# brade31919/radar_depth

Hardware: AMD Instinct MI355X
Metric: training samples/sec, resnet18_latefusion b=16 450x800 rgbd, 1/2/4/8 MI355X (higher is better)
Workload: dtype f32

## Files before the change

radar_depth_amd/csrc/gconv_split.hip:

```cpp
#include <math.h>
#include <stdlib.h>

#include <mutex>
#include <string>
#include <type_traits>
#include <unordered_map>
#include <vector>

#include "common.h"
#include "slot_map.h"

namespace rd {

typedef __bf16 sbf16x8 __attribute__((ext_vector_type(8)));
typedef unsigned int su32x4 __attribute__((ext_vector_type(4)));

constexpr unsigned GS_OOB = 0x80000000u;
constexpr int GS_CKP = 16;
constexpr int GS_PSB = (GS_CKP + 8) * 2;
constexpr int GS_UPP = 6;
constexpr int GS_UW = 2;
constexpr int GS_TPS = 3;

struct GsArgs {
    RdConvDesc d;
    const float* in;
    const unsigned short* w;
    float* out;
    const float* addend;
    const float* bias;
    float* stat;
    int act, act_cols, ld_add, ldw;
    int TH, TW, PP, tiles_total, n_cotiles, taps_max;
    int vec4;
    int pplane;
    long long wplane;
    int tapoff[RD_MAX_PHASES][RD_MAX_TAPS];
    unsigned long long* trace;
    int trace_role;
    const unsigned short* inp;
    long long xplane;
    long long mpix;
    int kplane;
    int stagger;
    int dbg;
    int ppitch[RD_MAX_PHASES];
    const int* slots;
    const float* bnb_x;
    const float* bnb_scale;
    const float* bnb_shift;
    const float* bnb_mean;
    int bnb_ld, bnb_act;
};

__device__ __forceinline__ void vm_wait_upto(int n) {
#define RD_VMW(k) case k: asm volatile("s_waitcnt vmcnt(" #k ") lgkmcnt(0)" ::: "memory"); break;
    switch (n < 47 ? n : 47) {
        RD_VMW(0) RD_VMW(1) RD_VMW(2) RD_VMW(3) RD_VMW(4) RD_VMW(5) RD_VMW(6) RD_VMW(7) RD_VMW(8) RD_VMW(9) RD_VMW(10) RD_VMW(11)
        RD_VMW(12) RD_VMW(13) RD_VMW(14) RD_VMW(15) RD_VMW(16) RD_VMW(17) RD_VMW(18) RD_VMW(19) RD_VMW(20) RD_VMW(21) RD_VMW(22) RD_VMW(23)
        RD_VMW(24) RD_VMW(25) RD_VMW(26) RD_VMW(27) RD_VMW(28) RD_VMW(29) RD_VMW(30) RD_VMW(31) RD_VMW(32) RD_VMW(33) RD_VMW(34) RD_VMW(35)
        RD_VMW(36) RD_VMW(37) RD_VMW(38) RD_VMW(39) RD_VMW(40) RD_VMW(41) RD_VMW(42) RD_VMW(43) RD_VMW(44) RD_VMW(45) RD_VMW(46) RD_VMW(47)
    }
#undef RD_VMW
}

typedef float sf32x2 __attribute__((ext_vector_type(2)));
typedef __bf16 sbf16x2 __attribute__((ext_vector_type(2)));
__device__ __forceinline__ unsigned cvt_pk(float a, float b) {
    sf32x2 v;
    v[0] = a; v[1] = b;
    return __builtin_bit_cast(unsigned, __builtin_convertvector(v, sbf16x2));
}
__device__ __forceinline__ void split8(const float4 v0, const float4 v1, sbf16x8& p0, sbf16x8& p1, sbf16x8& p2) {
    const float x[8] = {v0.x, v0.y, v0.z, v0.w, v1.x, v1.y, v1.z, v1.w};
    su32x4 w0, w1, w2;
#pragma unroll
    for (int i = 0; i < 4; ++i) {
        float a = x[2 * i], b = x[2 * i + 1];
        const unsigned u0 = cvt_pk(a, b);
        a -= __uint_as_float(u0 << 16);
        b -= __uint_as_float(u0 & 0xffff0000u);
        const unsigned u1 = cvt_pk(a, b);
        a -= __uint_as_float(u1 << 16);
        b -= __uint_as_float(u1 & 0xffff0000u);
        w0[i] = u0;
        w1[i] = u1;
        w2[i] = cvt_pk(a, b);
    }
    p0 = __builtin_bit_cast(sbf16x8, w0);
    p1 = __builtin_bit_cast(sbf16x8, w1);
    p2 = __builtin_bit_cast(sbf16x8, w2);
}

template <int MT, int NT, bool PDB, bool PRE, bool BNB = false>
__global__ __launch_bounds__(512) void gconv_split_kernel(const GsArgs a) {
    static_assert(!PRE || PDB, "the pre-split form copies the next chunk's patch while the current one is read: two patch buffers");
    constexpr int BM = 4 * MT * 32;
    constexpr int BN = NT * 32;
    constexpr int LBN = NT == 2 ? 6 : 5;
    extern __shared__ __attribute__((aligned(16))) float smem[];
    const int tid = threadIdx.x, lane = tid & 63;
    const int wave = __builtin_amdgcn_readfirstlane(tid >> 6);
    const bool loader = wave >= 4;
    const int wm = wave & 3;
    const int l31 = lane & 31, hh = lane >> 5;
    const RdConvDesc& D = a.d;

    if (a.trace && tid == 0) a.trace[(size_t)blockIdx.x * 64 + 62] = __builtin_readcyclecounter();
    const int vid = xcd_remap(blockIdx.x, gridDim.x);
    const int cot = vid % a.n_cotiles;
    const int pt = vid / a.n_cotiles;
    const int n = pt / a.tiles_total;
    const int tt = pt - n * a.tiles_total;
    int ph_ = 0;
    for (int i = 1; i < D.n_phases; ++i)
        if (tt >= D.phase[i].tile_begin) ph_ = i;
    const int ph = __builtin_amdgcn_readfirstlane(ph_);
    const RdPhase& P = D.phase[ph];
    const int tloc = tt - P.tile_begin;
    const int tiles_w = (P.lw + a.TW - 1) / a.TW;
    const int r0 = (tloc / tiles_w) * a.TH, c0 = (tloc % tiles_w) * a.TW;
    const int th_n = min(a.TH, P.lh - r0), tw_n = min(a.TW, P.lw - c0);
    const int IS = D.in_stride, OS = D.out_stride;
    const int PW = (a.TW - 1) * IS + (P.dw_max - P.dw_min) + 1;
    const int PWP = a.ppitch[ph];
    const int PH = (th_n - 1) * IS + (P.dh_max - P.dh_min) + 1;
    const int ih0 = r0 * IS + P.dh_min, iw0 = c0 * IS + P.dw_min;
    const int ntaps = __builtin_amdgcn_readfirstlane(P.n_taps);
    const int ngroups = (ntaps + GS_TPS - 1) / GS_TPS;
    const int co0 = cot * BN;

    int* s_opix = reinterpret_cast<int*>(smem);
    int* s_apix = s_opix + BM;
    int* s_widx = s_apix + BM;
    char* s_w = reinterpret_cast<char*>(s_widx + 32);
    constexpr int WPP = GS_TPS * 2 * BN * 16;
    constexpr int SLAB = 3 * WPP;
    char* s_patch = s_w + 3 * SLAB;
    const int pplane = a.pplane;

    for (int m = tid; m < BM; m += 512) {
        const int sv = a.slots[ph * BM + m];
        const bool have = sv >= 0;
        const int r = sv >> 16, c = sv & 0xffff, rho = -1 - sv;
        const bool ok = have && (r < th_n) && (c < tw_n);
        s_opix[m] = ok ? ((n * D.Ho + (r0 + r) * OS + P.out_off_h) * D.Wo + (c0 + c) * OS + P.out_off_w) : -1;
        s_apix[m] = have ? ((r * IS) * PWP + c * IS) : rho * IS;
    }
    if (tid < ntaps) s_widx[tid] = P.widx[tid];
    if constexpr (PRE) {
        const int n16 = (2 * 3 * pplane) >> 4;
        for (int e = tid; e < n16; e += 512) *reinterpret_cast<uint4*>(s_patch + (size_t)e * 16) = make_uint4(0u, 0u, 0u, 0u);
    }
    rd_sync();

    f32x16 acc[MT][NT];

    const int nchunks = D.Cin / GS_CKP;
    const int total_groups = nchunks * ngroups;
    const char* in_n = reinterpret_cast<const char*>(a.in) + (size_t)n * D.Hi * D.Wi * D.ldi * 4;
    const unsigned img_bytes = (unsigned)(D.Hi * D.Wi * D.ldi) * 4u;
    const int rowu = PW * 2;
    const int nseg = (rowu + 63) >> 6;
    const int nsegs = PH * nseg;
    auto unit_of = [&](int seg, unsigned& goff, int& ldst) {
        const int row = nseg == 1 ? seg : seg / nseg;
        const int cu = ((seg - row * nseg) << 6) + lane;
        const int px = cu >> 1, qq = cu & 1;
        const int ih = ih0 + row, iw = iw0 + px;
        const bool ok = seg < nsegs && cu < rowu;
        ldst = ok ? (row * PWP + px) * GS_PSB + qq * 16 : -1;
        goff = (ok && ih >= 0 && ih < D.Hi && iw >= 0 && iw < D.Wi) ? (unsigned)(((ih * D.Wi + iw) * D.ldi + qq * 8) * 4) : GS_OOB;
    };
    auto stage_first_chunk = [&]() {
        constexpr int UP8 = (GS_UPP + 1) / 2;
        const __amdgpu_buffer_rsrc_t r = __builtin_amdgcn_make_buffer_rsrc(const_cast<char*>(in_n), 0, img_bytes, 0x00020000);
        float4 f0[UP8], f1[UP8];
        int dst[UP8];
#pragma unroll
        for (int u = 0; u < UP8; ++u) {
            unsigned go;
            unit_of(wave + 8 * u, go, dst[u]);
            f0[u] = __builtin_bit_cast(float4, __builtin_amdgcn_raw_buffer_load_b128(r, (int)go, 0, 0));
            f1[u] = __builtin_bit_cast(float4, __builtin_amdgcn_raw_buffer_load_b128(r, (int)go + 16, 0, 0));
        }
        const unsigned base = (unsigned)(size_t)s_patch;
#pragma unroll
        for (int u = 0; u < UP8; ++u) {
            sbf16x8 q0, q1, q2;
            split8(f0[u], f1[u], q0, q1, q2);
            if (dst[u] >= 0) {
                const su32x4 d0 = __builtin_bit_cast(su32x4, q0), d1 = __builtin_bit_cast(su32x4, q1), d2 = __builtin_bit_cast(su32x4, q2);
                const unsigned ad = base + dst[u];
                asm volatile("ds_write_b128 %0, %1" ::"v"(ad), "v"(d0) : "memory");
                asm volatile("ds_write_b128 %0, %1" ::"v"(ad + pplane), "v"(d1) : "memory");
                asm volatile("ds_write_b128 %0, %1" ::"v"(ad + 2 * pplane), "v"(d2) : "memory");
            }
            __builtin_amdgcn_sched_barrier(0);
        }
    };

    if (loader) {
        const int ltid = tid - 256;
        const int lw = wave - 4;
        const int cin8 = D.Cin >> 3;
        unsigned pgo[GS_UPP];
        int pdst[GS_UPP];
        if constexpr (!PRE) {
#pragma unroll
            for (int u = 0; u < GS_UPP; ++u) unit_of(lw + 4 * u, pgo[u], pdst[u]);
        }
        auto issue_patch = [&](int pbuf, int blk) -> int {
            int cnt = 0;
            if (a.dbg & 8) return 0;
            const char* src0 = reinterpret_cast<const char*>(a.inp) + ((size_t)blk * a.mpix + (size_t)n * D.Hi * D.Wi) * 32;
            char* dst0 = s_patch + pbuf * 3 * pplane;
            const int nsg = (PW + 63) >> 6;
            for (int r = lw; r < PH; r += 4) {
                const int ih = ih0 + r;
                if (ih < 0 || ih >= D.Hi) continue;
                for (int sg = 0; sg < nsg; ++sg) {
                    const int col = (sg << 6) + lane, iw = iw0 + col;
                    const bool ok = col < PW && iw >= 0 && iw < D.Wi;
                    if (!__any(ok)) continue;
                    const char* src = src0 + ((size_t)ih * D.Wi + iw) * 32;
                    char* dst = dst0 + ((size_t)r * PWP + (sg << 6)) * 16;
                    if (ok) {
#pragma unroll
                        for (int p = 0; p < 3; ++p)
#pragma unroll
                            for (int u = 0; u < 2; ++u)
                                glds16(reinterpret_cast<const float*>(src + p * a.xplane + u * 16), reinterpret_cast<float*>(dst + p * pplane + u * a.kplane));
                    }
                    cnt += 6;
                }
            }
            return cnt;
        };
        auto issue_slab = [&](int buf, int cb, int g) -> int {
            if (a.dbg & 4) return 0;
            int cnt = 0;
            const int tap0 = g * GS_TPS;
            constexpr int welems = (GS_TPS * 2) << LBN;
            const char* src = reinterpret_cast<const char*>(a.w) + (size_t)(cb >> 3) * a.ldw * 16;
            char* dst = s_w + buf * SLAB;
#pragma unroll
            for (int u = 0; u < GS_UW; ++u) {
                const int e = ltid + u * 256;
                if (e < welems) {
                    const int j = e & (BN - 1), tk = e >> LBN;
                    const int k8 = tk & 1, t = tap0 + (tk >> 1);
                    const bool live = t < ntaps && co0 + j < D.Cout;
                    if (__any(live)) cnt += 3;
                    if (live) {
                        const size_t go = (((size_t)s_widx[t] * cin8 + k8) * a.ldw + co0 + j) * 16;
#pragma unroll
                        for (int p = 0; p < 3; ++p)
                            glds16(reinterpret_cast<const float*>(src + p * a.wplane + go), reinterpret_cast<float*>(dst + p * WPP + (e - lane) * 16));
                    } else {
                        const su32x4 z = {0u, 0u, 0u, 0u};
#pragma unroll
                        for (int p = 0; p < 3; ++p) {
                            const unsigned ad = (unsigned)(size_t)(dst + p * WPP + e * 16);
                            asm volatile("ds_write_b128 %0, %1" ::"v"(ad), "v"(z) : "memory");
                        }
                    }
                }
            }
            return cnt;
        };
        sbf16x8 pc[GS_UPP][3];
        float4 v0[GS_UPP], v1[GS_UPP];
        auto fetch = [&](int cb) {
            const __amdgpu_buffer_rsrc_t r = __builtin_amdgcn_make_buffer_rsrc(const_cast<char*>(in_n + cb * 4), 0, img_bytes - cb * 4, 0x00020000);
#pragma unroll
            for (int u = 0; u < GS_UPP; ++u) {
                v0[u] = __builtin_bit_cast(float4, __builtin_amdgcn_raw_buffer_load_b128(r, (int)pgo[u], 0, 0));
                v1[u] = __builtin_bit_cast(float4, __builtin_amdgcn_raw_buffer_load_b128(r, (int)pgo[u] + 16, 0, 0));
            }
        };
        auto split_units = [&](auto u0_, auto u1_) {
#pragma unroll
            for (int u = decltype(u0_)::value; u < decltype(u1_)::value; ++u) {
                split8(v0[u], v1[u], pc[u][0], pc[u][1], pc[u][2]);
                __builtin_amdgcn_sched_barrier(0);
            }
        };
        auto put_units = [&](int pbuf, auto u0_, auto u1_) {
            const unsigned base = (unsigned)(size_t)(s_patch + pbuf * 3 * pplane);
#pragma unroll
            for (int u = decltype(u0_)::value; u < decltype(u1_)::value; ++u)
                if (pdst[u] >= 0) {
#pragma unroll
                    for (int p = 0; p < 3; ++p) {
                        const unsigned addr = base + p * pplane + pdst[u];
                        const su32x4 dv = __builtin_bit_cast(su32x4, pc[u][p]);
                        asm volatile("ds_write_b128 %0, %1" ::"v"(addr), "v"(dv) : "memory");
                    }
                }
        };
        constexpr std::integral_constant<int, 0> U0{};
        constexpr std::integral_constant<int, GS_UPP> UN{};
        issue_slab(0, 0, 0);
        if (total_groups > 1) issue_slab(1, ngroups > 1 ? 0 : GS_CKP, ngroups > 1 ? 1 : 0);
        if constexpr (PRE) {
            auto lbarrier = [&]() {
                asm volatile("s_waitcnt lgkmcnt(0)" ::: "memory");
                __builtin_amdgcn_s_barrier();
                asm volatile("" ::: "memory");
            };
            issue_patch(0, 0);
            asm volatile("s_waitcnt vmcnt(0) lgkmcnt(0)" ::: "memory");
            int it = 0, wi = 2, c2 = 0, g2 = 2;
            while (g2 >= ngroups) { g2 -= ngroups; ++c2; }
            unsigned long long* ltr = (a.trace && a.trace_role == 2 && tid == 256) ? a.trace + (size_t)blockIdx.x * 64 : nullptr;
            for (int c = 0; c < nchunks; ++c) {
                for (int g = 0; g < ngroups; ++g, ++it) {
                    if (ltr && it < 30) ltr[2 * it] = __builtin_readcyclecounter();
                    lbarrier();
                    if (ltr && it < 30) ltr[2 * it + 1] = __builtin_readcyclecounter();
                    int n_now = 0;
                    if (it + 2 < total_groups) n_now += issue_slab(wi, c2 * GS_CKP, g2);
                    wi = wi == 2 ? 0 : wi + 1;
                    if (++g2 == ngroups) { g2 = 0; ++c2; }
                    if (g == 0 && c + 1 < nchunks) n_now += issue_patch((c + 1) & 1, c + 1);
                    vm_wait_upto(ngroups > 1 ? n_now : 0);
                }
            }
        } else {
        stage_first_chunk();
        const bool defer_fetch = ngroups >= 3;
        if (nchunks > 1 && !defer_fetch) {
            fetch(GS_CKP);
            asm volatile("s_waitcnt vmcnt(%0) lgkmcnt(0)" ::"n"(2 * GS_UPP) : "memory");
        } else {
            glds_wait();
        }
        int it = 0, wi = 2;
        int c2 = 0, g2 = 2;
        while (g2 >= ngroups) { g2 -= ngroups; ++c2; }
        const int gsplit = ngroups > 2 ? 1 : 0;
        unsigned long long* ltr = (a.trace && a.trace_role == 2 && tid == 256) ? a.trace + (size_t)blockIdx.x * 64 : nullptr;
        for (int c = 0; c < nchunks; ++c) {
            const bool more = c + 1 < nchunks;
            for (int g = 0; g < ngroups; ++g, ++it) {
                if (ltr && it < 30) ltr[2 * it] = __builtin_readcyclecounter();
                asm volatile("s_waitcnt lgkmcnt(0)" ::: "memory");
                __builtin_amdgcn_s_barrier();
                asm volatile("" ::: "memory");
                if (ltr && it < 30) ltr[2 * it + 1] = __builtin_readcyclecounter();
                if (it + 2 < total_groups) issue_slab(wi, c2 * GS_CKP, g2);
                wi = wi == 2 ? 0 : wi + 1;
                if (++g2 == ngroups) { g2 = 0; ++c2; }
                const bool first_fetch = it == 0 && nchunks > 1 && defer_fetch;
                const bool refetch = (g == ngroups - 1 && c + 2 < nchunks) || first_fetch;
                if (more) {
                    if (g == gsplit) split_units(U0, UN);
                    if (g == ngroups - 1) {
                        if constexpr (!PDB) {
                            asm volatile("s_waitcnt lgkmcnt(0)" ::: "memory");
                            __builtin_amdgcn_s_barrier();
                            asm volatile("" ::: "memory");
                        }
                        put_units(PDB ? ((c + 1) & 1) : 0, U0, UN);
                    }
                }
                if (refetch) fetch(first_fetch ? GS_CKP : (c + 2) * GS_CKP);
                if (refetch) asm volatile("s_waitcnt vmcnt(%0) lgkmcnt(0)" ::"n"(2 * GS_UPP) : "memory");
                else glds_wait();
            }
        }
        }
    } else {
        if constexpr (!PRE) stage_first_chunk();
#pragma unroll
        for (int mt = 0; mt < MT; ++mt)
#pragma unroll
            for (int nt = 0; nt < NT; ++nt)
#pragma unroll
                for (int i = 0; i < 16; ++i) acc[mt][nt][i] = 0.f;
        int aoffB[MT];
#pragma unroll
        for (int mt = 0; mt < MT; ++mt)
            aoffB[mt] = PRE ? s_apix[(wm * MT + mt) * 32 + l31] * 16 + hh * a.kplane : s_apix[(wm * MT + mt) * 32 + l31] * GS_PSB + hh * 16;
        const int boffB = (hh * BN + l31) * 16;
        const int tapv = a.tapoff[ph][lane < ntaps ? lane : 0];
        int abase[3][MT];
#pragma unroll
        for (int p = 0; p < 3; ++p)
#pragma unroll
            for (int mt = 0; mt < MT; ++mt) abase[p][mt] = p * pplane + aoffB[mt];
        auto load = [&](const char* pbase, const char* wbuf, int tap, int t, sbf16x8 (&A)[3][MT], sbf16x8 (&B)[3][NT]) {
            const int ao = __builtin_amdgcn_readlane(tapv, tap);
            const char* pa = pbase + ao;
            const char* wbl = wbuf + boffB;
#pragma unroll
            for (int p = 0; p < 3; ++p) {
#pragma unroll
                for (int mt = 0; mt < MT; ++mt) A[p][mt] = *reinterpret_cast<const sbf16x8*>(pa + abase[p][mt]);
#pragma unroll
                for (int nt = 0; nt < NT; ++nt) B[p][nt] = *reinterpret_cast<const sbf16x8*>(wbl + p * WPP + t * 2 * BN * 16 + nt * 512);
            }
        };
        auto loadA = [&](const char* pbase, int tap, sbf16x8 (&A)[3][MT]) {
            const char* pa = pbase + __builtin_amdgcn_readlane(tapv, tap);
#pragma unroll
            for (int p = 0; p < 3; ++p)
#pragma unroll
                for (int mt = 0; mt < MT; ++mt) A[p][mt] = *reinterpret_cast<const sbf16x8*>(pa + abase[p][mt]);
        };
        auto loadB = [&](const char* wbuf, int t, sbf16x8 (&B)[3][NT]) {
            const char* wbl = wbuf + boffB;
#pragma unroll
            for (int p = 0; p < 3; ++p)
#pragma unroll
                for (int nt = 0; nt < NT; ++nt) B[p][nt] = *reinterpret_cast<const sbf16x8*>(wbl + p * WPP + t * 2 * BN * 16 + nt * 512);
        };
        auto interleave = [&]() {
#pragma unroll
            for (int i = 0; i < 3 * (MT + NT); ++i) {
                __builtin_amdgcn_sched_group_barrier(0x008, 2, 0);
                __builtin_amdgcn_sched_group_barrier(0x002, 1, 0);
                __builtin_amdgcn_sched_group_barrier(0x100, 1, 0);
            }
            __builtin_amdgcn_sched_group_barrier(0x008, 6 * MT * NT - 6 * (MT + NT), 0);
        };
        auto mma = [&](const sbf16x8 (&A)[3][MT], const sbf16x8 (&B)[3][NT]) {
#pragma unroll
            for (int mt = 0; mt < MT; ++mt)
#pragma unroll
                for (int nt = 0; nt < NT; ++nt) {
                    f32x16 c = acc[mt][nt];
                    RD_SPLIT_TERMS(c, A[0][mt], A[1][mt], A[2][mt], B[0][nt], B[1][nt], B[2][nt])
                    acc[mt][nt] = c;
                }
        };
        sbf16x8 fa[2][3][MT], fb[2][3][NT];
        unsigned long long* trc = (a.trace && a.trace_role == 1 && tid == 0) ? a.trace + (size_t)blockIdx.x * 64 : nullptr;
        int it = 0, wi = 0, c = 0, g = 0;
        bool have = false;
        auto group = [&](auto parity) {
            constexpr int P0 = decltype(parity)::value, P1 = 1 - P0;
            if (trc && it < 30) trc[2 * it] = __builtin_readcyclecounter();
            rd_sync();
            if (trc && it < 30) trc[2 * it + 1] = __builtin_readcyclecounter();
            const char* pbase = s_patch + (PDB ? (c & 1) * 3 * pplane : 0);
            const int wn = wi == 2 ? 0 : wi + 1;
            const char* wb = s_w + wi * SLAB;
            const char* wbn = s_w + wn * SLAB;
            const int tap0 = g * GS_TPS;
            const bool pref = g + 1 < ngroups;
            if constexpr (PRE && MT == 3 && NT == 2) {
                if (!have) loadA(pbase, min(tap0, ntaps - 1), fa[0]);
                loadB(wb, 0, fb[0]);
            } else if constexpr (MT == 3 && NT == 2) {
                if (!have) { loadA(pbase, min(tap0, ntaps - 1), fa[0]); loadB(wb, 0, fb[P0]); }
            } else {
                if (!have) load(pbase, wb, min(tap0, ntaps - 1), 0, fa[P0], fb[P0]);
                else if constexpr (PRE) loadB(wb, 0, fb[P0]);
            }
            __builtin_amdgcn_sched_barrier(0);
            if constexpr (MT == 3 && NT == 2) {
                auto rstep = [&](sbf16x8 (&A)[3][MT], const sbf16x8 (&Bc)[3][NT], sbf16x8 (&Bn)[3][NT], int tapn, const char* wnext, int tn, bool doA, bool doB) {
                    const char* pa = pbase + __builtin_amdgcn_readlane(tapv, tapn);
                    const char* wbl = wnext + boffB;
#pragma unroll
                    for (int mt = 0; mt < MT; ++mt)
#pragma unroll
                        for (int nt = 0; nt < NT; ++nt) {
                            f32x16 c = acc[mt][nt];
                            RD_SPLIT_TERMS(c, A[0][mt], A[1][mt], A[2][mt], Bc[0][nt], Bc[1][nt], Bc[2][nt])
                            acc[mt][nt] = c;
                            __builtin_amdgcn_sched_barrier(0);
                            if (nt == 0) {
                                if (doB) {
#pragma unroll
                                    for (int q = 2 * mt; q < 2 * mt + 2; ++q)
                                        Bn[q / NT][q % NT] = *reinterpret_cast<const sbf16x8*>(wbl + (q / NT) * WPP + tn * 2 * BN * 16 + (q % NT) * 512);
                                }
                            } else if (doA) {
#pragma unroll
                                for (int pp = 0; pp < 3; ++pp) A[pp][mt] = *reinterpret_cast<const sbf16x8*>(pa + abase[pp][mt]);
                            }
                            __builtin_amdgcn_sched_barrier(0);
                        }
                };
                if constexpr (PRE) {
                    rstep(fa[0], fb[0], fb[1], min(tap0 + 1, ntaps - 1), wb, 1, true, true);
                    rstep(fa[0], fb[1], fb[0], min(tap0 + 2, ntaps - 1), wb, 2, true, true);
                    rstep(fa[0], fb[0], fb[1], min(tap0 + 3, ntaps - 1), wb, 0, pref, false);
                } else {
                    rstep(fa[0], fb[P0], fb[P1], min(tap0 + 1, ntaps - 1), wb, 1, true, true);
                    rstep(fa[0], fb[P1], fb[P0], min(tap0 + 2, ntaps - 1), wb, 2, true, true);
                    rstep(fa[0], fb[P0], fb[P1], min(tap0 + 3, ntaps - 1), wbn, 0, pref, pref);
                }
            } else if constexpr (MT * NT < 4 || (MT * NT == 4 && PDB)) {
                load(pbase, wb, min(tap0 + 1, ntaps - 1), 1, fa[P1], fb[P1]);
                mma(fa[P0], fb[P0]);
                interleave();
                __builtin_amdgcn_sched_barrier(0);
                load(pbase, wb, min(tap0 + 2, ntaps - 1), 2, fa[P0], fb[P0]);
                mma(fa[P1], fb[P1]);
                interleave();
                __builtin_amdgcn_sched_barrier(0);
                if (pref) {
                    if constexpr (PRE) loadA(pbase, min(tap0 + 3, ntaps - 1), fa[P1]);
                    else load(pbase, wbn, min(tap0 + 3, ntaps - 1), 0, fa[P1], fb[P1]);
                    mma(fa[P0], fb[P0]);
                    interleave();
                } else {
                    mma(fa[P0], fb[P0]);
                }
            } else {
                load(pbase, wb, min(tap0 + 1, ntaps - 1), 1, fa[P1], fb[P1]);
                __builtin_amdgcn_sched_barrier(0);
                mma(fa[P0], fb[P0]);
                __builtin_amdgcn_sched_barrier(0);
                load(pbase, wb, min(tap0 + 2, ntaps - 1), 2, fa[P0], fb[P0]);
                __builtin_amdgcn_sched_barrier(0);
                mma(fa[P1], fb[P1]);
                __builtin_amdgcn_sched_barrier(0);
                if (pref) {
                    if constexpr (PRE) loadA(pbase, min(tap0 + 3, ntaps - 1), fa[P1]);
                    else load(pbase, wbn, min(tap0 + 3, ntaps - 1), 0, fa[P1], fb[P1]);
                }
                __builtin_amdgcn_sched_barrier(0);
                mma(fa[P0], fb[P0]);
            }
            __builtin_amdgcn_sched_barrier(0);
            have = pref;
            wi = wn;
            if constexpr (!PDB) {
                if (!pref && c + 1 < nchunks) rd_sync();
            }
            ++it;
            if (++g == ngroups) { g = 0; ++c; }
        };
        while (it + 2 <= total_groups) {
            group(std::integral_constant<int, 0>{});
            group(std::integral_constant<int, 1>{});
        }
        if (it < total_groups) group(std::integral_constant<int, 0>{});
        if (trc) { trc[60] = __builtin_readcyclecounter(); trc[63] = (unsigned long long)total_groups; }
    }

    float ssum[NT], ssq[NT];
#pragma unroll
    for (int nt = 0; nt < NT; ++nt) ssum[nt] = ssq[nt] = 0.f;
    if (!loader && !(a.dbg & 16)) {
        const bool has_add = a.addend != nullptr;
        const bool has_bias = a.bias != nullptr;
        const int cob = co0 + l31;
        float biasv[NT];
#pragma unroll
        for (int nt = 0; nt < NT; ++nt) biasv[nt] = (has_bias && cob + nt * 32 < D.Cout) ? a.bias[cob + nt * 32] : 0.f;
        const bool want_stat = a.stat != nullptr;
        const int q4l = l31 & 3, k4l = l31 >> 2;
        const bool odd1 = q4l & 1, odd2 = q4l & 2;
        float4 ssum4[NT], ssq4[NT];
#pragma unroll
        for (int nt = 0; nt < NT; ++nt) ssum4[nt] = ssq4[nt] = make_float4(0.f, 0.f, 0.f, 0.f);
        bool any4 = false;
#pragma unroll
        for (int mt = 0; mt < MT; ++mt) {
            int ro4[4];
            bool rok4[4];
#pragma unroll
            for (int g = 0; g < 4; ++g) {
                ro4[g] = s_opix[(wm * MT + mt) * 32 + q4l + 8 * g + 4 * hh];
                rok4[g] = ro4[g] >= 0;
                ro4[g] = rok4[g] ? ro4[g] : 0;
            }
            if (a.vec4) {
                any4 = true;
                const int cq = co0 + 4 * k4l;
                float4 addv[NT][4];
                float4 bS[NT], bT[NT], bM[NT];
                if constexpr (BNB) {
#pragma unroll
                    for (int nt = 0; nt < NT; ++nt) {
                        const bool on = cq + nt * 32 < D.Cout;
                        bS[nt] = on ? ld4(a.bnb_scale + cq + nt * 32) : make_float4(0.f, 0.f, 0.f, 0.f);
                        bT[nt] = on ? ld4(a.bnb_shift + cq + nt * 32) : make_float4(0.f, 0.f, 0.f, 0.f);
                        bM[nt] = on ? ld4(a.bnb_mean + cq + nt * 32) : make_float4(0.f, 0.f, 0.f, 0.f);
                    }
                }
                if (has_add || BNB) {
#pragma unroll
                    for (int g = 0; g < 4; ++g) {
                        const float* ap = BNB ? a.bnb_x + (size_t)ro4[g] * a.bnb_ld + cq : a.addend + (size_t)ro4[g] * a.ld_add + cq;
#pragma unroll
                        for (int nt = 0; nt < NT; ++nt) addv[nt][g] = (cq + nt * 32 < D.Cout) ? ld4(ap + nt * 32) : make_float4(0.f, 0.f, 0.f, 0.f);
                    }
                }
#pragma unroll
                for (int nt = 0; nt < NT; ++nt) {
                    const bool cok4 = cq + nt * 32 < D.Cout;
                    float4 b4 = make_float4(0.f, 0.f, 0.f, 0.f);
                    if (has_bias && cok4) b4 = *reinterpret_cast<const float4*>(a.bias + cq + nt * 32);
#pragma unroll
                    for (int g = 0; g < 4; ++g) {
                        float e0 = acc[mt][nt][4 * g], e1 = acc[mt][nt][4 * g + 1], e2 = acc[mt][nt][4 * g + 2], e3 = acc[mt][nt][4 * g + 3];
                        quad_transpose(e0, e1, e2, e3, odd1, odd2);
                        float4 v = make_float4(e0 + b4.x, e1 + b4.y, e2 + b4.z, e3 + b4.w);
                        if (has_add && !BNB) { v.x += addv[nt][g].x; v.y += addv[nt][g].y; v.z += addv[nt][g].z; v.w += addv[nt][g].w; }
                        const int cc = cq + nt * 32;
                        if (cc < a.act_cols) {
                            v.x = act_fwd(v.x, a.act); v.y = act_fwd(v.y, a.act); v.z = act_fwd(v.z, a.act); v.w = act_fwd(v.w, a.act);
                        }
                        if (cok4 && rok4[g]) st4(a.out + (size_t)ro4[g] * D.ldo + cc, v);
                        if (want_stat && rok4[g]) {
                            if constexpr (BNB) {
                                const float4 xv = addv[nt][g];
                                const float gx = v.x * act_grad_from_out(fmaf(bS[nt].x, xv.x, bT[nt].x), a.bnb_act);
                                const float gy = v.y * act_grad_from_out(fmaf(bS[nt].y, xv.y, bT[nt].y), a.bnb_act);
                                const float gz = v.z * act_grad_from_out(fmaf(bS[nt].z, xv.z, bT[nt].z), a.bnb_act);
                                const float gw = v.w * act_grad_from_out(fmaf(bS[nt].w, xv.w, bT[nt].w), a.bnb_act);
                                ssum4[nt].x += gx; ssum4[nt].y += gy; ssum4[nt].z += gz; ssum4[nt].w += gw;
                                ssq4[nt].x += gx * (xv.x - bM[nt].x); ssq4[nt].y += gy * (xv.y - bM[nt].y);
                                ssq4[nt].z += gz * (xv.z - bM[nt].z); ssq4[nt].w += gw * (xv.w - bM[nt].w);
                            } else {
                                ssum4[nt].x += v.x; ssum4[nt].y += v.y; ssum4[nt].z += v.z; ssum4[nt].w += v.w;
                                ssq4[nt].x += v.x * v.x; ssq4[nt].y += v.y * v.y; ssq4[nt].z += v.z * v.z; ssq4[nt].w += v.w * v.w;
                            }
                        }
                    }
                }
            } else {
                int ro[16];
#pragma unroll
                for (int i = 0; i < 16; ++i) ro[i] = s_opix[(wm * MT + mt) * 32 + (i & 3) + 8 * (i >> 2) + 4 * hh];
#pragma unroll
                for (int nt = 0; nt < NT; ++nt) {
                    const int co = cob + nt * 32;
                    const bool cok = co < D.Cout;
// ... 337 lines not shown
                        const int cc = cq + nt * 32;
                        if (cc < a.act_cols) {
                            v.x = act_fwd(v.x, a.act); v.y = act_fwd(v.y, a.act); v.z = act_fwd(v.z, a.act); v.w = act_fwd(v.w, a.act);
                        }
                        if (cok4 && rok4[q]) st4(a.out + (size_t)ro4[q] * D.ldo + cc, v);
                        if (want_stat && rok4[q]) {
                            if constexpr (BNB) {
                                const float4 xv = addv[nt][q];
                                const float gx = v.x * act_grad_from_out(fmaf(bS[nt].x, xv.x, bT[nt].x), a.bnb_act);
                                const float gy = v.y * act_grad_from_out(fmaf(bS[nt].y, xv.y, bT[nt].y), a.bnb_act);
                                const float gz = v.z * act_grad_from_out(fmaf(bS[nt].z, xv.z, bT[nt].z), a.bnb_act);
                                const float gw = v.w * act_grad_from_out(fmaf(bS[nt].w, xv.w, bT[nt].w), a.bnb_act);
                                ssum4[nt].x += gx; ssum4[nt].y += gy; ssum4[nt].z += gz; ssum4[nt].w += gw;
                                ssq4[nt].x += gx * (xv.x - bM[nt].x); ssq4[nt].y += gy * (xv.y - bM[nt].y);
                                ssq4[nt].z += gz * (xv.z - bM[nt].z); ssq4[nt].w += gw * (xv.w - bM[nt].w);
                            } else {
                                ssum4[nt].x += v.x; ssum4[nt].y += v.y; ssum4[nt].z += v.z; ssum4[nt].w += v.w;
                                ssq4[nt].x += v.x * v.x; ssq4[nt].y += v.y * v.y; ssq4[nt].z += v.z * v.z; ssq4[nt].w += v.w * v.w;
                            }
                        }
                    }
                }
            } else {
                int ro[16];
#pragma unroll
                for (int i = 0; i < 16; ++i) ro[i] = s_opix[(wm * MT + mt) * 32 + (i & 3) + 8 * (i >> 2) + 4 * hh];
#pragma unroll
                for (int nt = 0; nt < NT; ++nt) {
                    const int co = cob + nt * 32;
                    const bool cok = co < D.Cout;
#pragma unroll
                    for (int i = 0; i < 16; ++i) {
                        if (cok && ro[i] >= 0) {
                            float v = acc[mt][nt][i] + biasv[nt];
                            if (has_add) v += a.addend[(size_t)ro[i] * a.ld_add + co];
                            if (co < a.act_cols) v = act_fwd(v, a.act);
                            a.out[(size_t)ro[i] * D.ldo + co] = v;
                            ssum[nt] += v;
                            ssq[nt] += v * v;
                        }
                    }
                }
            }
        }
        if (want_stat && __any(any4)) {
#pragma unroll
            for (int nt = 0; nt < NT; ++nt) {
                float4 s4 = ssum4[nt], q4 = ssq4[nt];
                s4.x += dpp_xor1(s4.x); s4.y += dpp_xor1(s4.y); s4.z += dpp_xor1(s4.z); s4.w += dpp_xor1(s4.w);
                q4.x += dpp_xor1(q4.x); q4.y += dpp_xor1(q4.y); q4.z += dpp_xor1(q4.z); q4.w += dpp_xor1(q4.w);
                s4.x += dpp_xor2(s4.x); s4.y += dpp_xor2(s4.y); s4.z += dpp_xor2(s4.z); s4.w += dpp_xor2(s4.w);
                q4.x += dpp_xor2(q4.x); q4.y += dpp_xor2(q4.y); q4.z += dpp_xor2(q4.z); q4.w += dpp_xor2(q4.w);
                ssum[nt] += odd2 ? (odd1 ? s4.w : s4.z) : (odd1 ? s4.y : s4.x);
                ssq[nt] += odd2 ? (odd1 ? q4.w : q4.z) : (odd1 ? q4.y : q4.x);
            }
        }
    }
    if (a.stat) {
        rd_sync();
        float* red = reinterpret_cast<float*>(s_w);
#pragma unroll
        for (int nt = 0; nt < NT; ++nt) {
            const float s = ssum[nt] + __shfl_xor(ssum[nt], 32, 64);
            const float q = ssq[nt] + __shfl_xor(ssq[nt], 32, 64);
            if (hh == 0) {
                red[(wm * 2 + 0) * BN + nt * 32 + l31] = s;
                red[(wm * 2 + 1) * BN + nt * 32 + l31] = q;
            }
        }
        rd_sync();
        if (tid < 2 * BN) {
            const int which = tid / BN, j = tid - which * BN;
            float s = 0.f;
#pragma unroll
            for (int w = 0; w < 4; ++w) s += red[(w * 2 + which) * BN + j];
            const int co = co0 + j;
            if (co < D.Cout) a.stat[((size_t)pt * (BNB ? 3 : 2) + which) * D.Cout + co] = s;
        }
    }
    if (a.trace && a.trace_role == 1 && tid == 0) {
        a.trace[(size_t)blockIdx.x * 64 + 61] = __builtin_readcyclecounter();
        a.trace[(size_t)blockIdx.x * 64 + 58] = __builtin_amdgcn_s_memrealtime();
    }
}

struct GsPlan {
    int MT, NT, TH, TW, PP, tiles_total, n_cotiles, taps_max, pplane;
    size_t lds_bytes;
    int pdb;
    int sp2;
    int ppitch[RD_MAX_PHASES];
    unsigned nres[RD_MAX_PHASES][4];
};

static int gs_pick_pitch(const RdConvDesc& d, const RdPhase& p, int TH, int TW, int G, unsigned (*nres)[4]) {
    const int PW = (TW - 1) * d.in_stride + (p.dw_max - p.dw_min) + 1;
    int best = PW, best_over = -1, n[16];
    for (int pad = 0; pad < 4; ++pad) {
        const int over = gs_residues(TH, TW, PW + pad, G, n);
        if (best_over < 0 || over < best_over) { best_over = over; best = PW + pad; }
        if (over == 0) break;
    }
    if (nres) {
        gs_residues(TH, TW, best, G, n);
        for (int w = 0; w < 4; ++w) {
            (*nres)[w] = 0;
            for (int b = 0; b < 4; ++b) (*nres)[w] |= (unsigned)(n[4 * w + b] > 255 ? 255 : n[4 * w + b]) << (8 * b);
        }
    }
    return best;
}

static int gs_patch_pixels(const RdConvDesc& d, const RdPhase& p, int TH, int TW, int G, int* rows, int* cols) {
    const int th = TH < p.lh ? TH : p.lh;
    const int PH = (th - 1) * d.in_stride + (p.dh_max - p.dh_min) + 1;
    const int PW = (TW - 1) * d.in_stride + (p.dw_max - p.dw_min) + 1;
    if (rows) *rows = PH;
    if (cols) *cols = PW;
    return PH * gs_pick_pitch(d, p, TH, TW, G, nullptr);
}

static void gs_fill_slot_map(const RdConvDesc& d, GsPlan& pl) {
    const int G = 4 * pl.MT * 32 / 16;
    for (int i = 0; i < RD_MAX_PHASES; ++i) {
        pl.ppitch[i] = 0;
        for (int w = 0; w < 4; ++w) pl.nres[i][w] = 0;
    }
    for (int i = 0; i < d.n_phases; ++i) pl.ppitch[i] = gs_pick_pitch(d, d.phase[i], pl.TH, pl.TW, G, &pl.nres[i]);
}

static bool plan_gconv_split(const RdConvDesc& d, GsPlan& best, bool pre) {
    struct Cfg { int MT, NT; };
    static const Cfg cfgs[] = {{3, 2}, {2, 2}, {1, 2}, {2, 1}, {1, 1}};
    int taps_max = 0;
    for (int i = 0; i < d.n_phases; ++i) {
        taps_max = taps_max > d.phase[i].n_taps ? taps_max : d.phase[i].n_taps;
    }
    int pr = 0;
    for (int i = 1; i < d.n_phases; ++i)
        if ((int64_t)d.phase[i].lh * d.phase[i].lw > (int64_t)d.phase[pr].lh * d.phase[pr].lw) pr = i;
    const RdPhase& P = d.phase[pr];
    double best_cost = -1;
    static const char* force = getenv("RD_GCONV_SPLIT_FORCE");
    int cfg_i = -1;
    for (const Cfg& c : cfgs) {
        ++cfg_i;
        if (force && atoi(force) != cfg_i) continue;
        const int BM = 4 * c.MT * 32, BN = c.NT * 32;
        if (BN > 32 && d.Cout <= 32) continue;
        const int n_cot = cdiv(d.Cout, BN);
        for (int twt = 1; twt <= cdiv(P.lw, 4); ++twt) {
            const int TW = cdiv(P.lw, twt);
            if (TW > BM) continue;
            int TH = BM / TW;
            if (TH > P.lh) TH = P.lh;
            TH = cdiv(P.lh, cdiv(P.lh, TH));
            int PP = 0, segs = 0;
            for (int i = 0; i < d.n_phases; ++i) {
                int rows, cols;
                const int pp = gs_patch_pixels(d, d.phase[i], TH, TW, BM / 16, &rows, &cols);
                PP = PP > pp ? PP : pp;
                const int sg = rows * cdiv(cols * 2, 64);
                segs = segs > sg ? segs : sg;
            }
            if (!pre && segs > 4 * GS_UPP) continue;
            if (pre && 6 * segs > 4 * 44) continue;
            const int pplane = pre ? 2 * (((PP * 16) + 63) & ~63) : ((((PP + 1) * GS_PSB) + 15) & ~15);
            static const char* nopdb = getenv("RD_GCONV_SPLIT_NOPDB");
            for (int pdb = (nopdb && !pre) ? 0 : 1; pdb >= (pre ? 1 : 0); --pdb) {
                const size_t lds = (size_t)(2 * BM + 32) * 4 + (size_t)3 * 3 * GS_TPS * 2 * BN * 16 + (size_t)(pdb ? 2 : 1) * 3 * pplane + 64;
                if (lds > 160 * 1024 - 512) continue;
                double groups = 0, wgs = 0;
                for (int i = 0; i < d.n_phases; ++i) {
                    const double t = (double)cdiv(d.phase[i].lh, TH) * cdiv(d.phase[i].lw, TW);
                    groups += t * cdiv(d.phase[i].n_taps, GS_TPS);
                    wgs += t;
                }
                const double groups_per_wg = groups / wgs;
                wgs *= (double)d.N * n_cot;
                const double mfma_clk = 3.0 * c.MT * c.NT * 6 * 42;
                const double lds_clk = 3.0 * 3 * (c.MT + c.NT) * 4 * 4 / 0.7;
                const double per_group = (mfma_clk > lds_clk ? mfma_clk : lds_clk) + 1300.0;
                const double per_chunk = groups_per_wg * per_group;
                const double per_wg = (double)(d.Cin / GS_CKP) * per_chunk + 7000.0 + 16.0 * c.MT * c.NT * 60;
                const double rounds = ceil(wgs / (double)num_cus());
                const double cost = rounds * per_wg;
                if (best_cost < 0 || cost < best_cost) {
                    best_cost = cost;
                    best = GsPlan{c.MT, c.NT, TH, TW, PP, 0, n_cot, taps_max, pplane, lds, pdb, 0, {}, {}};
                }
                break;
            }
        }
    }
    return best_cost > 0;
}

static bool plan_sp2(const RdConvDesc& d, GsPlan& best) {
    struct Cfg { int MT, NT; };
    static const Cfg cfgs[] = {{2, 2}, {1, 2}, {2, 1}, {1, 1}, {3, 1}};
    int taps_max = 0;
    for (int i = 0; i < d.n_phases; ++i) taps_max = taps_max > d.phase[i].n_taps ? taps_max : d.phase[i].n_taps;
    int pr = 0;
    for (int i = 1; i < d.n_phases; ++i)
        if ((int64_t)d.phase[i].lh * d.phase[i].lw > (int64_t)d.phase[pr].lh * d.phase[pr].lw) pr = i;
    const RdPhase& P = d.phase[pr];
    double best_cost = -1;
    static const char* force = getenv("RD_GCONV_SP2_FORCE");
    int cfg_i = -1;
    for (const Cfg& c : cfgs) {
        ++cfg_i;
        if (force && atoi(force) != cfg_i) continue;
        const int BM = 4 * c.MT * 32, BN = c.NT * 32;
        if (BN > 32 && d.Cout <= 32) continue;
        const int n_cot = cdiv(d.Cout, BN);
        for (int twt = 1; twt <= cdiv(P.lw, 4); ++twt) {
            const int TW = cdiv(P.lw, twt);
            if (TW > BM) continue;
            int TH = BM / TW;
            if (TH > P.lh) TH = P.lh;
            TH = cdiv(P.lh, cdiv(P.lh, TH));
            int PP = 0;
            double copies = 0;
            for (int i = 0; i < d.n_phases; ++i) {
                int rows, cols;
                const int pp = gs_patch_pixels(d, d.phase[i], TH, TW, BM / 16, &rows, &cols);
                PP = PP > pp ? PP : pp;
                copies = copies > 6.0 * rows * cdiv(cols, 64) ? copies : 6.0 * rows * cdiv(cols, 64);
            }
            const int pplane = 2 * (((PP * 16) + 63) & ~63);
            const size_t lds = (size_t)(2 * BM + 32) * 4 + (size_t)2 * 3 * GS_TPS * 2 * BN * 16 + (size_t)3 * pplane + 64;
            if (lds > 80 * 1024 - 256) continue;
            double groups = 0, wgs = 0;
            for (int i = 0; i < d.n_phases; ++i) {
                const double t = (double)cdiv(d.phase[i].lh, TH) * cdiv(d.phase[i].lw, TW);
                groups += t * cdiv(d.phase[i].n_taps, GS_TPS);
                wgs += t;
            }
            const double groups_per_wg = groups / wgs;
            wgs *= (double)d.N * n_cot;
            const double per_group = 3.0 * c.MT * c.NT * 6 * 34 + 250.0;
            const double per_chunk = groups_per_wg * per_group + 600.0 + copies / 4 * 40.0;
            const double per_wg = (double)(d.Cin / GS_CKP) * per_chunk + 3000.0 + 16.0 * c.MT * c.NT * 50;
            const double per_cu = ceil(wgs / (double)num_cus());
            const double cost = per_cu * per_wg + (((int)per_cu & 1) ? 0.5 * per_wg : 0.0);
            if (best_cost < 0 || cost < best_cost) {
                best_cost = cost;
                best = GsPlan{c.MT, c.NT, TH, TW, PP, 0, n_cot, taps_max, pplane, lds, 0, 1, {}, {}};
            }
        }
    }
    return best_cost > 0;
}

template <int MT, int NT, int DBG = 0, bool BNB = false>
static int launch_sp2(const GsArgs& a, int grid, size_t lds, hipStream_t s) {
    static std::atomic<unsigned long long> attr_set{0};
    auto k = gconv_sp2_kernel<MT, NT, DBG, BNB>;
    RD_SET_ATTR_ONCE(attr_set, hipFuncSetAttribute(reinterpret_cast<const void*>(k), hipFuncAttributeMaxDynamicSharedMemorySize, 80 * 1024));
    hipLaunchKernelGGL(k, dim3(grid), dim3(256), lds, s, a);
    RD_CHECK_LAUNCH("gconv_sp2_kernel");
    return RD_OK;
}

template <int MT, int NT, bool PDB, bool PRE, bool BNB = false>
static int launch_gs(const GsArgs& a, int grid, size_t lds, hipStream_t s) {
    static std::atomic<unsigned long long> attr_set{0};
    auto k = gconv_split_kernel<MT, NT, PDB, PRE, BNB>;
    RD_SET_ATTR_ONCE(attr_set, hipFuncSetAttribute(reinterpret_cast<const void*>(k), hipFuncAttributeMaxDynamicSharedMemorySize, 160 * 1024));
    hipLaunchKernelGGL(k, dim3(grid), dim3(512), lds, s, a);
    RD_CHECK_LAUNCH("gconv_split_kernel");
    return RD_OK;
}

static std::mutex g_gs_mu;
static int g_gs_all = -1;
static unsigned g_gs_epoch = 0;
static bool gs_plan_all() {
    std::lock_guard<std::mutex> lk(g_gs_mu);
    if (g_gs_all < 0) g_gs_all = getenv("RD_GCONV_SPLIT_ALL") ? 1 : 0;
    return g_gs_all == 1;
}

static bool gs_shape_ok(const RdConvDesc* d, bool sp2 = false) {
    if (!d || d->n_phases < 1 || d->n_phases > RD_MAX_PHASES) return false;
    if (d->Cin % 16 != 0 || d->ldi % 4 != 0 || d->Cin < 32 || d->Cout < 32) return false;
    if (d->in_stride < 1 || d->in_stride > 2 || d->out_stride < 1 || d->out_stride > 2) return false;
    if (!gs_plan_all()) {
        int taps_max = 0;
        for (int i = 0; i < d->n_phases; ++i) taps_max = taps_max > d->phase[i].n_taps ? taps_max : d->phase[i].n_taps;
        if (taps_max < 4) return false;
        if (!sp2 && (d->Cin < 64 || d->Cout < 64)) return false;
        static const int s2pre = getenv("RD_GCONV_S2_PRE") ? atoi(getenv("RD_GCONV_S2_PRE")) : 2;
        if (d->in_stride == 2 && taps_max <= 9 && !(sp2 && s2pre >= 1)) return false;
        if (d->out_stride == 2 && taps_max <= 4 && !(sp2 && s2pre >= 2)) return false;
    }
    if ((int64_t)d->Hi * d->Wi * d->ldi * 4 >= (int64_t)GS_OOB) return false;
    for (int i = 0; i < d->n_phases; ++i) {
        const RdPhase& p = d->phase[i];
        if (p.n_taps < 1 || p.n_taps > RD_MAX_TAPS || p.lh < 1 || p.lw < 1) return false;
        for (int t = 0; t < p.n_taps; ++t)
            if (p.dh[t] < p.dh_min || p.dh[t] > p.dh_max || p.dw[t] < p.dw_min || p.dw[t] > p.dw_max) return false;
    }
    return true;
}

static int gs_plan_query(const RdConvDesc* d, GsPlan& pl, RdConvDesc& dd, bool pre = false) {
    struct Entry { int ok; GsPlan pl; RdConvDesc dd; };
    static std::mutex mu;
    static std::unordered_map<std::string, Entry> cache;
    static unsigned cache_epoch = 0;
    if (!d) return 0;
    std::string key(reinterpret_cast<const char*>(d), sizeof(RdConvDesc));
    key.push_back(pre ? 'P' : 'R');
    {
        unsigned ep;
        { std::lock_guard<std::mutex> lk(g_gs_mu); ep = g_gs_epoch; }
        std::lock_guard<std::mutex> lk(mu);
        if (ep != cache_epoch) { cache.clear(); cache_epoch = ep; }
        auto it = cache.find(key);
        if (it != cache.end()) { pl = it->second.pl; dd = it->second.dd; return it->second.ok; }
    }
    Entry e{};
    e.dd = *d;
    static const char* no_sp2 = getenv("RD_GCONV_SP2");
    const bool sp2 = pre && !(no_sp2 && atoi(no_sp2) == 0);
    e.ok = gs_shape_ok(d, sp2) && (sp2 ? plan_sp2(e.dd, e.pl) : plan_gconv_split(e.dd, e.pl, pre)) ? 1 : 0;
    if (e.ok) {
        int tb = 0;
        for (int i = 0; i < e.dd.n_phases; ++i) {
            e.dd.phase[i].tile_begin = tb;
            tb += cdiv(e.dd.phase[i].lh, e.pl.TH) * cdiv(e.dd.phase[i].lw, e.pl.TW);
        }
        e.pl.tiles_total = tb;
        gs_fill_slot_map(e.dd, e.pl);
    }
    pl = e.pl; dd = e.dd;
    std::lock_guard<std::mutex> lk(mu);
    cache.emplace(std::move(key), e);
    return e.ok;
}

static const int* gs_slot_table(const RdConvDesc* d, bool pre, const GsPlan& pl) {
    static std::mutex mu;
// ... 289 lines not shown
```

Measured before the change: 1085.

## Swizzle split-conv LDS patch layout and prefer double-buffered tile heights

Drops the 8-channel padding from each LDS patch pixel and replaces it with an XOR swizzle on the half-pixel offset to avoid bank conflicts, aligning the patch base and planes to 256 bytes. The smaller pixel pitch lets larger tiles fit, and the planner now also tries a shorter tile height so double buffering of the patch fits, charging single-buffer plans an extra per-chunk cost. The risks are mismatched swizzling between the stage and read paths and extra address arithmetic on every A-fragment load.

```diff
diff --git a/radar_depth_amd/csrc/gconv_split.hip b/radar_depth_amd/csrc/gconv_split.hip
--- a/radar_depth_amd/csrc/gconv_split.hip
+++ b/radar_depth_amd/csrc/gconv_split.hip
@@ -17,7 +17,8 @@
 
 constexpr unsigned GS_OOB = 0x80000000u;
 constexpr int GS_CKP = 16;
-constexpr int GS_PSB = (GS_CKP + 8) * 2;
+constexpr int GS_PSB = GS_CKP * 2;
+constexpr int GS_PAL = 256;
 constexpr int GS_UPP = 6;
 constexpr int GS_UW = 2;
 constexpr int GS_TPS = 3;
@@ -53,6 +54,13 @@
     int bnb_ld, bnb_act;
 };
 
+__host__ __device__ constexpr int gs_patch_off(int idx, int h) { return idx * GS_PSB + ((h ^ ((idx >> 3) & 1)) << 4); }
+__device__ __forceinline__ int gs_patch_swz(int s) { return s ^ ((s >> 4) & 16); }
+__host__ __device__ constexpr int gs_patch_base(int BM, int BN, bool pre) {
+    const int raw = (2 * BM + 32) * 4 + 3 * 3 * GS_TPS * 2 * BN * 16;
+    return pre ? raw : (raw + GS_PAL - 1) / GS_PAL * GS_PAL;
+}
+
 __device__ __forceinline__ void vm_wait_upto(int n) {
 #define RD_VMW(k) case k: asm volatile("s_waitcnt vmcnt(" #k ") lgkmcnt(0)" ::: "memory"); break;
     switch (n < 47 ? n : 47) {
@@ -136,7 +144,7 @@
     char* s_w = reinterpret_cast<char*>(s_widx + 32);
     constexpr int WPP = GS_TPS * 2 * BN * 16;
     constexpr int SLAB = 3 * WPP;
-    char* s_patch = s_w + 3 * SLAB;
+    char* s_patch = reinterpret_cast<char*>(smem) + gs_patch_base(BM, BN, PRE);
     const int pplane = a.pplane;
 
     for (int m = tid; m < BM; m += 512) {
@@ -169,7 +177,7 @@
         const int px = cu >> 1, qq = cu & 1;
         const int ih = ih0 + row, iw = iw0 + px;
         const bool ok = seg < nsegs && cu < rowu;
-        ldst = ok ? (row * PWP + px) * GS_PSB + qq * 16 : -1;
+        ldst = ok ? gs_patch_off(row * PWP + px, qq) : -1;
         goff = (ok && ih >= 0 && ih < D.Hi && iw >= 0 && iw < D.Wi) ? (unsigned)(((ih * D.Wi + iw) * D.ldi + qq * 8) * 4) : GS_OOB;
     };
     auto stage_first_chunk = [&]() {
@@ -390,6 +398,10 @@
         for (int p = 0; p < 3; ++p)
 #pragma unroll
             for (int mt = 0; mt < MT; ++mt) abase[p][mt] = p * pplane + aoffB[mt];
+        auto afrag = [&](const char* pa, int ao, int p, int mt) -> const sbf16x8* {
+            if constexpr (PRE) return reinterpret_cast<const sbf16x8*>(pa + abase[p][mt]);
+            else return reinterpret_cast<const sbf16x8*>(pa - ao + gs_patch_swz(aoffB[mt] + ao) + p * pplane);
+        };
         auto load = [&](const char* pbase, const char* wbuf, int tap, int t, sbf16x8 (&A)[3][MT], sbf16x8 (&B)[3][NT]) {
             const int ao = __builtin_amdgcn_readlane(tapv, tap);
             const char* pa = pbase + ao;
@@ -397,17 +409,18 @@
 #pragma unroll
             for (int p = 0; p < 3; ++p) {
 #pragma unroll
-                for (int mt = 0; mt < MT; ++mt) A[p][mt] = *reinterpret_cast<const sbf16x8*>(pa + abase[p][mt]);
+                for (int mt = 0; mt < MT; ++mt) A[p][mt] = *afrag(pa, ao, p, mt);
 #pragma unroll
                 for (int nt = 0; nt < NT; ++nt) B[p][nt] = *reinterpret_cast<const sbf16x8*>(wbl + p * WPP + t * 2 * BN * 16 + nt * 512);
             }
         };
         auto loadA = [&](const char* pbase, int tap, sbf16x8 (&A)[3][MT]) {
-            const char* pa = pbase + __builtin_amdgcn_readlane(tapv, tap);
+            const int ao = __builtin_amdgcn_readlane(tapv, tap);
+            const char* pa = pbase + ao;
 #pragma unroll
             for (int p = 0; p < 3; ++p)
 #pragma unroll
-                for (int mt = 0; mt < MT; ++mt) A[p][mt] = *reinterpret_cast<const sbf16x8*>(pa + abase[p][mt]);
+                for (int mt = 0; mt < MT; ++mt) A[p][mt] = *afrag(pa, ao, p, mt);
         };
         auto loadB = [&](const char* wbuf, int t, sbf16x8 (&B)[3][NT]) {
             const char* wbl = wbuf + boffB;
@@ -462,7 +475,8 @@
             __builtin_amdgcn_sched_barrier(0);
             if constexpr (MT == 3 && NT == 2) {
                 auto rstep = [&](sbf16x8 (&A)[3][MT], const sbf16x8 (&Bc)[3][NT], sbf16x8 (&Bn)[3][NT], int tapn, const char* wnext, int tn, bool doA, bool doB) {
-                    const char* pa = pbase + __builtin_amdgcn_readlane(tapv, tapn);
+                    const int ao = __builtin_amdgcn_readlane(tapv, tapn);
+                    const char* pa = pbase + ao;
                     const char* wbl = wnext + boffB;
 #pragma unroll
                     for (int mt = 0; mt < MT; ++mt)
@@ -480,7 +494,7 @@
                                 }
                             } else if (doA) {
 #pragma unroll
-                                for (int pp = 0; pp < 3; ++pp) A[pp][mt] = *reinterpret_cast<const sbf16x8*>(pa + abase[pp][mt]);
+                                for (int pp = 0; pp < 3; ++pp) A[pp][mt] = *afrag(pa, ao, pp, mt);
                             }
                             __builtin_amdgcn_sched_barrier(0);
                         }
@@ -1124,9 +1138,13 @@
         for (int twt = 1; twt <= cdiv(P.lw, 4); ++twt) {
             const int TW = cdiv(P.lw, twt);
             if (TW > BM) continue;
-            int TH = BM / TW;
-            if (TH > P.lh) TH = P.lh;
-            TH = cdiv(P.lh, cdiv(P.lh, TH));
+            int TH0 = BM / TW;
+            if (TH0 > P.lh) TH0 = P.lh;
+            TH0 = cdiv(P.lh, cdiv(P.lh, TH0));
+            bool fits_twice = false;
+            for (int alt = 0; alt < (pre ? 1 : 2) && !fits_twice; ++alt) {
+            const int TH = alt == 0 ? TH0 : cdiv(P.lh, cdiv(P.lh, TH0) + 1);
+            if (alt == 1 && TH == TH0) break;
             int PP = 0, segs = 0;
             for (int i = 0; i < d.n_phases; ++i) {
                 int rows, cols;
@@ -1135,13 +1153,15 @@
                 const int sg = rows * cdiv(cols * 2, 64);
                 segs = segs > sg ? segs : sg;
             }
-            if (!pre && segs > 4 * GS_UPP) continue;
-            if (pre && 6 * segs > 4 * 44) continue;
-            const int pplane = pre ? 2 * (((PP * 16) + 63) & ~63) : ((((PP + 1) * GS_PSB) + 15) & ~15);
+            if (!pre && segs > 4 * GS_UPP) break;
+            if (pre && 6 * segs > 4 * 44) break;
+            const int pplane = pre ? 2 * (((PP * 16) + 63) & ~63) : ((((PP + 1) * GS_PSB) + GS_PAL - 1) & ~(GS_PAL - 1));
             static const char* nopdb = getenv("RD_GCONV_SPLIT_NOPDB");
-            for (int pdb = (nopdb && !pre) ? 0 : 1; pdb >= (pre ? 1 : 0); --pdb) {
-                const size_t lds = (size_t)(2 * BM + 32) * 4 + (size_t)3 * 3 * GS_TPS * 2 * BN * 16 + (size_t)(pdb ? 2 : 1) * 3 * pplane + 64;
+            if (nopdb && !pre && alt == 1) break;
+            for (int pdb = (nopdb && !pre) ? 0 : 1; pdb >= (pre || alt == 1 ? 1 : 0); --pdb) {
+                const size_t lds = (size_t)gs_patch_base(BM, BN, pre) + (size_t)(pdb ? 2 : 1) * 3 * pplane + 64;
                 if (lds > 160 * 1024 - 512) continue;
+                fits_twice |= pdb == 1;
                 double groups = 0, wgs = 0;
                 for (int i = 0; i < d.n_phases; ++i) {
                     const double t = (double)cdiv(d.phase[i].lh, TH) * cdiv(d.phase[i].lw, TW);
@@ -1153,7 +1173,7 @@
                 const double mfma_clk = 3.0 * c.MT * c.NT * 6 * 42;
                 const double lds_clk = 3.0 * 3 * (c.MT + c.NT) * 4 * 4 / 0.7;
                 const double per_group = (mfma_clk > lds_clk ? mfma_clk : lds_clk) + 1300.0;
-                const double per_chunk = groups_per_wg * per_group;
+                const double per_chunk = groups_per_wg * per_group + (pdb ? 0.0 : 1200.0);
                 const double per_wg = (double)(d.Cin / GS_CKP) * per_chunk + 7000.0 + 16.0 * c.MT * c.NT * 60;
                 const double rounds = ceil(wgs / (double)num_cus());
                 const double cost = rounds * per_wg;
@@ -1162,6 +1182,7 @@
                     best = GsPlan{c.MT, c.NT, TH, TW, PP, 0, n_cot, taps_max, pplane, lds, pdb, 0, {}, {}};
                 }
                 break;
+            }
             }
         }
     }
```

Result: no change. 1090, median of 6 (+0.5%).
